# mattiaskvist/yolo-v1

Measured on AMD Instinct MI355X. Metric: images/sec at 448x448, forward (YOLOv1Backbone + FC head), higher is better.
Workload: dtype bf16; 1 GPU; BASELINE.json configs[1]: batch=64/GPU 448x448 forward-only, YOLOv1Backbone + FC head, 1xMI355X per rank; global_batch=64, per_gpu_batch=64, weights=random init (torch default, seed 0), parallelism=single

## Files before the change

include/yolo_hip.h:

```cpp
#ifndef YOLO_HIP_H
#define YOLO_HIP_H

#include <stddef.h>
#include <stdint.h>

#ifdef __cplusplus
extern "C" {
#endif

#define YOLO_HIP_ABI_VERSION 2

#define YOLO_E_ARG (-1)
#define YOLO_E_UNSUPPORTED (-2)

typedef void *yolo_stream_t;

int yolo_hip_abi_version(void);
const char *yolo_hip_last_error(void);
int yolo_debug_stamps(void *buf, int k_iter);
int yolo_stream_create(int low, yolo_stream_t *out);


int yolo_decode(const float *pred, int N, int S, int B, int C, double conf_thr,
                double *rec, int32_t *counts, yolo_stream_t stream);
// ... 91 lines not shown
int yolo_maxpool2_bwd_codes(const yolo_pool_desc *d, const void *ypool_bf16, const void *codes_u16, const void *dpool_bf16,
                            float slope, void *dz_bf16, yolo_stream_t stream);


int yolo_nchw_f32_to_nhwc_bf16(const float *x, int N, int C, int H, int W, void *y, int Cpad,
                               int halo_lo, int halo_hi, yolo_stream_t stream);
int yolo_nhwc_bf16_to_nchw_f32(const void *x, int N, int C, int H, int W, int halo, float *y, yolo_stream_t stream);
int yolo_nhwc_bf16_to_nchw_bf16(const void *x, int N, int C, int H, int W, int halo, void *y, yolo_stream_t stream);

int yolo_pack_conv_weight(const float *w_oihw, int Cout, int Cin, int KH, int KW, int Cinp, int KWp,
                          void *w_fwd_bf16, void *w_dgrad_bf16, yolo_stream_t stream);
int yolo_pack_fc_weight(const float *w, int O, int C, int HW, void *w_fwd_bf16, void *w_t_bf16, yolo_stream_t stream);
int yolo_pack_fc_weight_blocked(const float *w, int O, long K, void *w_panels_bf16, yolo_stream_t stream);
int yolo_pack_fc_weight_blocked_hwc(const float *w, int O, int C, int HW, void *w_panels_bf16, yolo_stream_t stream);
int yolo_unpack_conv_wgrad(const float *dw_packed, int Cout, int Cin, int KH, int KW, int Cinp, int KWp,
                           float *dw_oihw, int accumulate, yolo_stream_t stream);
int yolo_conv_stem7_fwd(const void *x_nhwc4_bf16, const void *w_packed_bf16, const float *bias, int N, int Ho, int Wo,
                        long x_img_stride, int x_row_stride, float slope, int pool2, void *out_bf16,
                        long out_img_stride, int out_row_stride, int out_off, void *out_full_bf16,
                        long full_img_stride, int full_row_stride, int full_off, yolo_stream_t stream);
int yolo_conv_stem7_fwd_f32(const float *x_nchw_f32, const void *w_packed_bf16, const float *bias, int N, int H, int W, float slope,
                            int pool2, void *out_bf16, long out_img_stride, int out_row_stride, int out_off, void *out_full_bf16,
                            long full_img_stride, int full_row_stride, int full_off, yolo_stream_t stream);
int yolo_wgrad_stem7(const void *x_nhwc4_bf16, const void *dy_bf16, int N, int Ho, int Wo, long x_img_stride,
                     int x_row_stride, long dy_img_stride, int dy_row_stride, int dy_off, float *dw_oihw,
                     float *db, float *scratch, long scratch_elems, yolo_stream_t stream);
int yolo_wgrad_stem7_pooled(const void *x_nhwc4_bf16, const void *y_full_bf16, int N, int Ho, int Wo, long x_img_stride,
                            int x_row_stride, long y_img_stride, int y_row_stride, int y_off, const void *dpool_bf16,
                            long dp_img_stride, int dp_row_stride, int dp_off, float slope, float *dw_oihw, float *db,
                            float *scratch, long scratch_elems, yolo_stream_t stream);
int yolo_wgrad_stem7_codes(const void *x_nhwc4_bf16, const void *y_pooled_bf16, const void *codes_u16, int N, int Ho, int Wo,
                           long x_img_stride, int x_row_stride, const void *dpool_bf16, long dp_img_stride, int dp_row_stride,
                           int dp_off, float slope, float *dw_oihw, float *db, float *scratch, long scratch_elems,
                           yolo_stream_t stream);
#define YOLO_PACK_MAX 32
typedef struct yolo_conv_pack_item {
    const float *w;
    void *w_fwd_bf16;
    void *w_dgrad_bf16;
    int Cout, Cin, KH, KW;
} yolo_conv_pack_item;
typedef struct yolo_conv_unpack_item {
    const float *dw_packed;
    float *dw_oihw;
    int Cout, Cin, KH, KW;
} yolo_conv_unpack_item;
// ... 122 lines not shown
```

yolo-v1_amd/csrc/stem.hip:

```cpp
#include <algorithm>

#include "common.h"

namespace yolo {

typedef __attribute__((ext_vector_type(8))) __bf16 sbf16x8;
typedef __attribute__((ext_vector_type(4))) float sf32x4;

#define STEM_GLDS16(gptr, lptr) \
    __builtin_amdgcn_global_load_lds((const __attribute__((address_space(1))) void *)(gptr), (__attribute__((address_space(3))) void *)(lptr), 16, 0, 0)

constexpr int SF_TH = 8, SF_TW = 16;
constexpr int SF_PW = 40, SF_PH = 21;
constexpr int SF_X_BYTES = 7 * 1024;
constexpr int SF_OP = 64 + 8;
constexpr int SF_OUT_BYTES = SF_TH * SF_TW * SF_OP * 2;

struct StemFwdParams {
    const bf16_t *x;
    const bf16_t *w;
    const float *bias;
    bf16_t *out;
    int tiles_x, tiles_y, ntiles;
    long x_img_stride, out_img_stride;
    int x_row_stride, out_row_stride, out_off;
    int pool;
    float slope;
    bf16_t *full;
    unsigned short *codes;
    long full_img_stride;
    int full_row_stride, full_off;
    const float *x32;
    int H, W;
};

template <bool F32IN>
__global__ void __launch_bounds__(256, 2) stem_fwd_kernel(const StemFwdParams p)
{
    __shared__ __attribute__((aligned(16))) char patchA[SF_X_BYTES];
    __shared__ __attribute__((aligned(16))) char patchB[SF_X_BYTES];
    __shared__ __attribute__((aligned(16))) bf16_t otileA[SF_TH * SF_TW * SF_OP];
    __shared__ __attribute__((aligned(16))) bf16_t otileB[SF_TH * SF_TW * SF_OP];
    const int tid = threadIdx.x, lane = tid & 63;
    const int wave = __builtin_amdgcn_readfirstlane(tid >> 6);
    const int n16 = lane & 15, kb = lane >> 4;

    sbf16x8 afrag[4][7];
#pragma unroll
    for (int mb = 0; mb < 4; ++mb)
#pragma unroll
        for (int ky = 0; ky < 7; ++ky)
            afrag[mb][ky] = *reinterpret_cast<const sbf16x8 *>(p.w + ((mb * 16 + n16) * 7 + ky) * 32 + kb * 8);
    float bias_r[4][4];
#pragma unroll
    for (int mb = 0; mb < 4; ++mb)
#pragma unroll
        for (int r = 0; r < 4; ++r) bias_r[mb][r] = p.bias[mb * 16 + 4 * kb + r];

    int x_off[2];
#pragma unroll
    for (int i = 0; i < 2; ++i) {
        int slot = (i * 4 + wave) * 64 + lane;
        if (slot >= SF_PH * (SF_PW / 2)) slot = SF_PH * (SF_PW / 2) - 1;
        x_off[i] = (slot / (SF_PW / 2)) * p.x_row_stride + (slot % (SF_PW / 2)) * 8;
    }
    auto stage = [&](char *sb, int tile) {
        const int tx = tile % p.tiles_x, r = tile / p.tiles_x;
        const int ty = r % p.tiles_y, n = r / p.tiles_y;
        const bf16_t *xb = p.x + (long)n * p.x_img_stride + (long)(ty * SF_TH * 2) * p.x_row_stride + tx * SF_TW * 2 * 4;
        STEM_GLDS16(xb + x_off[0], sb + wave * 1024);
        if (wave < 3) STEM_GLDS16(xb + x_off[1], sb + (4 + wave) * 1024);
    };

    constexpr int F32_ITEMS = SF_PH * 3 * 11, F32_PER_THREAD = (F32_ITEMS + 255) / 256;
    float4 xr[F32_PER_THREAD];
    if constexpr (F32IN) {
        for (int i = tid; i < SF_X_BYTES / 16; i += 256) {
            *reinterpret_cast<uint4 *>(patchA + i * 16) = uint4{0u, 0u, 0u, 0u};
            *reinterpret_cast<uint4 *>(patchB + i * 16) = uint4{0u, 0u, 0u, 0u};
        }
        __syncthreads();
    }
    auto f32_load = [&](int tile) {
        const int tx = tile % p.tiles_x, r = tile / p.tiles_x;
        const int ty = r % p.tiles_y, n = r / p.tiles_y;
        const float *xb = p.x32 + (long)n * 3 * p.H * p.W;
#pragma unroll
        for (int j = 0; j < F32_PER_THREAD; ++j) {
            const int item = j * 256 + tid;
            const int q = item % 11, rc = item / 11, c = rc % 3, pr = rc / 3;
            const int y = ty * SF_TH * 2 - 3 + pr, x = tx * SF_TW * 2 - 4 + 4 * q;
            const bool in = item < F32_ITEMS && y >= 0 && y < p.H && x >= 0 && x < p.W;
            xr[j] = in ? *reinterpret_cast<const float4 *>(xb + ((long)c * p.H + y) * p.W + x) : float4{0.0f, 0.0f, 0.0f, 0.0f};
        }
    };
    auto f32_store = [&](char *sb) {
#pragma unroll
        for (int j = 0; j < F32_PER_THREAD; ++j) {
            const int item = j * 256 + tid;
            if (item >= F32_ITEMS) continue;
            const int q = item % 11, rc = item / 11, c = rc % 3, pr = rc / 3;
            const float v[4] = {xr[j].x, xr[j].y, xr[j].z, xr[j].w};
#pragma unroll
            for (int e = 0; e < 4; ++e) {
                const int ppx = 4 * q - 1 + e;
                if (ppx >= 0 && ppx < SF_PW) *reinterpret_cast<bf16_t *>(sb + (pr * SF_PW + ppx) * 8 + c * 2) = f32_to_bf16(v[e]);
            }
        }
    };

    const int b_base = ((4 * wave) * SF_PW + 2 * n16 + 2 * kb) * 8;

    auto mfma_phase = [&](const char *sb, bf16_t *otile) {
        sf32x4 acc[4][2];
#pragma unroll
        for (int mb = 0; mb < 4; ++mb)
#pragma unroll
            for (int rr = 0; rr < 2; ++rr) acc[mb][rr] = sf32x4{0.0f, 0.0f, 0.0f, 0.0f};
#pragma unroll
        for (int ky = 0; ky < 7; ++ky) {
            sbf16x8 bfr[2];
#pragma unroll
            for (int rr = 0; rr < 2; ++rr) bfr[rr] = *reinterpret_cast<const sbf16x8 *>(sb + b_base + ((2 * rr + ky) * SF_PW) * 8);
#pragma unroll
            for (int mb = 0; mb < 4; ++mb)
#pragma unroll
                for (int rr = 0; rr < 2; ++rr) acc[mb][rr] = __builtin_amdgcn_mfma_f32_16x16x32_bf16(afrag[mb][ky], bfr[rr], acc[mb][rr], 0, 0, 0);
        }
#pragma unroll
        for (int rr = 0; rr < 2; ++rr) {
            const int px = (2 * wave + rr) * SF_TW + n16;
#pragma unroll
            for (int mb = 0; mb < 4; ++mb) {
                float v[4];
#pragma unroll
                for (int r = 0; r < 4; ++r) {
                    v[r] = acc[mb][rr][r] + bias_r[mb][r];
                    v[r] = v[r] > 0.0f ? v[r] : v[r] * p.slope;
                }
                uint2 o;
                o.x = (unsigned)f32_to_bf16(v[0]) | ((unsigned)f32_to_bf16(v[1]) << 16);
                o.y = (unsigned)f32_to_bf16(v[2]) | ((unsigned)f32_to_bf16(v[3]) << 16);
                *reinterpret_cast<uint2 *>(otile + px * SF_OP + mb * 16 + 4 * kb) = o;
            }
        }
    };
    auto store_phase = [&](const bf16_t *otile, int tile) {
        const int tx = tile % p.tiles_x, r0 = tile / p.tiles_x;
        const int ty = r0 % p.tiles_y, n = r0 / p.tiles_y;
        bf16_t *ob = p.out + (long)n * p.out_img_stride + p.out_off;
        if (p.pool) {
            const int c8 = tid & 7, q = tid >> 3, qy = q >> 3, qx = q & 7;
            const bf16_t *s0 = otile + ((2 * qy) * SF_TW + 2 * qx) * SF_OP + c8 * 8;
            const uint4 a = *reinterpret_cast<const uint4 *>(s0), b = *reinterpret_cast<const uint4 *>(s0 + SF_OP);
            const uint4 c = *reinterpret_cast<const uint4 *>(s0 + SF_TW * SF_OP), d = *reinterpret_cast<const uint4 *>(s0 + SF_TW * SF_OP + SF_OP);
            const unsigned va[4] = {a.x, a.y, a.z, a.w}, vb[4] = {b.x, b.y, b.z, b.w}, vc[4] = {c.x, c.y, c.z, c.w}, vd[4] = {d.x, d.y, d.z, d.w};
            unsigned o[4];
#pragma unroll
            for (int k = 0; k < 4; ++k) {
                const float lo = fmaxf(fmaxf(__uint_as_float(va[k] << 16), __uint_as_float(vb[k] << 16)), fmaxf(__uint_as_float(vc[k] << 16), __uint_as_float(vd[k] << 16)));
                const float hi = fmaxf(fmaxf(__uint_as_float(va[k] & 0xffff0000u), __uint_as_float(vb[k] & 0xffff0000u)),
                                       fmaxf(__uint_as_float(vc[k] & 0xffff0000u), __uint_as_float(vd[k] & 0xffff0000u)));
                o[k] = (__float_as_uint(lo) >> 16) | (__float_as_uint(hi) & 0xffff0000u);
            }
            const long pa = (long)(ty * (SF_TH / 2) + qy) * p.out_row_stride + (tx * (SF_TW / 2) + qx) * 64 + c8 * 8;
            *reinterpret_cast<uint4 *>(ob + pa) = uint4{o[0], o[1], o[2], o[3]};
            if (p.codes) {
                unsigned code = 0;
#pragma unroll
                for (int k = 0; k < 4; ++k) {
#pragma unroll
                    for (int hf = 0; hf < 2; ++hf) {
                        const float w0 = hf ? __uint_as_float(va[k] & 0xffff0000u) : __uint_as_float(va[k] << 16);
                        const float w1 = hf ? __uint_as_float(vb[k] & 0xffff0000u) : __uint_as_float(vb[k] << 16);
                        const float w2 = hf ? __uint_as_float(vc[k] & 0xffff0000u) : __uint_as_float(vc[k] << 16);
                        const float w3 = hf ? __uint_as_float(vd[k] & 0xffff0000u) : __uint_as_float(vd[k] << 16);
                        unsigned am = 0;
                        float m = w0;
                        if (w1 > m) { m = w1; am = 1; }
                        if (w2 > m) { m = w2; am = 2; }
                        if (w3 > m) { m = w3; am = 3; }
                        code |= am << (2 * (2 * k + hf));
                    }
                }
                p.codes[((long)n * p.out_img_stride + p.out_off + pa) >> 3] = (unsigned short)code;
            }
            if (p.full) {
                bf16_t *fb = p.full + (long)n * p.full_img_stride + p.full_off;
#pragma unroll
                for (int pass = 0; pass < 4; ++pass) {
                    const int idx = pass * 256 + tid, cc = idx & 7, px = idx >> 3;
                    const uint4 v = *reinterpret_cast<const uint4 *>(otile + px * SF_OP + cc * 8);
                    *reinterpret_cast<uint4 *>(fb + (long)(ty * SF_TH + (px >> 4)) * p.full_row_stride + (tx * SF_TW + (px & 15)) * 64 + cc * 8) = v;
                }
            }
        } else {
#pragma unroll
            for (int pass = 0; pass < 4; ++pass) {
                const int idx = pass * 256 + tid, c8 = idx & 7, px = idx >> 3;
                const int py = px >> 4, pxx = px & 15;
                const uint4 v = *reinterpret_cast<const uint4 *>(otile + px * SF_OP + c8 * 8);
                *reinterpret_cast<uint4 *>(ob + (long)(ty * SF_TH + py) * p.out_row_stride + (tx * SF_TW + pxx) * 64 + c8 * 8) = v;
            }
        }
    };

    const int G = gridDim.x;
    int tile = blockIdx.x, prev = -1;
    if (tile < p.ntiles) {
        if constexpr (F32IN) {
            f32_load(tile);
            f32_store(patchA);
        } else {
            stage(patchA, tile);
        }
    }
    while (tile < p.ntiles) {
        asm volatile("s_waitcnt vmcnt(0) lgkmcnt(0)" ::: "memory");
        __builtin_amdgcn_s_barrier();
        asm volatile("" ::: "memory");
        if (tile + G < p.ntiles) {
            if constexpr (F32IN) f32_load(tile + G);
            else stage(patchB, tile + G);
        }
        if (prev >= 0) store_phase(otileB, prev);
        mfma_phase(patchA, otileA);
        if constexpr (F32IN) {
            if (tile + G < p.ntiles) f32_store(patchB);
// ... 10 lines not shown
        asm volatile("s_waitcnt vmcnt(0) lgkmcnt(0)" ::: "memory");
        __builtin_amdgcn_s_barrier();
        asm volatile("" ::: "memory");
        if (tile + G < p.ntiles) {
            if constexpr (F32IN) f32_load(tile + G);
            else stage(patchA, tile + G);
        }
        store_phase(otileA, prev);
        mfma_phase(patchB, otileB);
        if constexpr (F32IN) {
            if (tile + G < p.ntiles) f32_store(patchA);
        }
        prev = tile;
        tile += G;
        if (tile >= p.ntiles) {
            asm volatile("s_waitcnt lgkmcnt(0)" ::: "memory");
            __builtin_amdgcn_s_barrier();
            asm volatile("" ::: "memory");
            store_phase(otileB, prev);
        }
    }
}

}

using namespace yolo;

YOLO_API int yolo_conv_stem7_fwd(const void *x_nhwc4, const void *w_packed, const float *bias, int N, int Ho, int Wo, long x_img_stride, int x_row_stride,
                                 float slope, int pool2, void *out, long out_img_stride, int out_row_stride, int out_off, void *out_full, long full_img_stride,
                                 int full_row_stride, int full_off, yolo_stream_t stream)
{
    if (pool2 == 3 && !out_full) return fail(YOLO_E_ARG, "yolo_conv_stem7_fwd: pool2 = 3 writes the arg-max codes through out_full");
    if (out_full && pool2 != 3 && (!pool2 || (full_row_stride & 7) || (full_img_stride & 7) || (full_off & 7) || ((uintptr_t)out_full & 15)))
        return fail(YOLO_E_ARG, "yolo_conv_stem7_fwd: out_full needs pool2 = 1 and strides in multiples of 8 elements");
    if (!x_nhwc4 || !w_packed || !bias || !out || N <= 0 || Ho <= 0 || Wo <= 0) return fail(YOLO_E_ARG, "yolo_conv_stem7_fwd: bad argument");
    if ((Ho % SF_TH) || (Wo % SF_TW)) return fail(YOLO_E_UNSUPPORTED, "yolo_conv_stem7_fwd: output %dx%d is not a multiple of %dx%d (use yolo_igemm)", Ho, Wo, SF_TH, SF_TW);
    if ((x_row_stride & 7) || (x_img_stride & 7) || (out_row_stride & 7) || (out_img_stride & 7) || (out_off & 7) || ((uintptr_t)x_nhwc4 & 15) || ((uintptr_t)out & 15) ||
        ((uintptr_t)w_packed & 15))
        return fail(YOLO_E_UNSUPPORTED, "yolo_conv_stem7_fwd: strides must be multiples of 8 elements and pointers 16-B aligned");
    StemFwdParams p{};
    p.x = (const bf16_t *)x_nhwc4; p.w = (const bf16_t *)w_packed; p.bias = bias; p.out = (bf16_t *)out;
    p.tiles_x = Wo / SF_TW; p.tiles_y = Ho / SF_TH;
    const long nt = (long)N * p.tiles_x * p.tiles_y;
    if (nt > 0x7fffffffL) return fail(YOLO_E_UNSUPPORTED, "yolo_conv_stem7_fwd: too many tiles");
    p.ntiles = (int)nt;
    p.x_img_stride = x_img_stride; p.out_img_stride = out_img_stride;
    p.x_row_stride = x_row_stride; p.out_row_stride = out_row_stride; p.out_off = out_off;
    p.pool = pool2 ? 1 : 0;
    p.slope = slope;
    if (pool2 == 3) {
        p.codes = (unsigned short *)out_full;
    } else {
        p.full = (bf16_t *)out_full; p.full_img_stride = full_img_stride; p.full_row_stride = full_row_stride; p.full_off = full_off;
    }
    const long G = std::min<long>(nt, 1024);
    hipLaunchKernelGGL(stem_fwd_kernel<false>, dim3((unsigned)G), dim3(256), 0, STRM(stream), p);
    return check_launch("yolo_conv_stem7_fwd");
}

YOLO_API int yolo_conv_stem7_fwd_f32(const float *x_nchw, const void *w_packed, const float *bias, int N, int H, int W, float slope, int pool2, void *out,
                                     long out_img_stride, int out_row_stride, int out_off, void *out_full, long full_img_stride, int full_row_stride, int full_off,
                                     yolo_stream_t stream)
{
    const int Ho = H / 2, Wo = W / 2;
    if (!x_nchw || !w_packed || !bias || !out || N <= 0 || H <= 0 || W <= 0 || (H & 1) || (W & 1)) return fail(YOLO_E_ARG, "yolo_conv_stem7_fwd_f32: bad argument");
    if (pool2 == 3 && !out_full) return fail(YOLO_E_ARG, "yolo_conv_stem7_fwd_f32: pool2 = 3 writes the arg-max codes through out_full");
    if (out_full && pool2 != 3 && (!pool2 || (full_row_stride & 7) || (full_img_stride & 7) || (full_off & 7) || ((uintptr_t)out_full & 15)))
        return fail(YOLO_E_ARG, "yolo_conv_stem7_fwd_f32: out_full needs pool2 = 1 and strides in multiples of 8 elements");
    if ((Ho % SF_TH) || (Wo % SF_TW)) return fail(YOLO_E_UNSUPPORTED, "yolo_conv_stem7_fwd_f32: output %dx%d is not a multiple of %dx%d", Ho, Wo, SF_TH, SF_TW);
    if ((uintptr_t)x_nchw & 15) return fail(YOLO_E_UNSUPPORTED, "yolo_conv_stem7_fwd_f32: the input must be 16-B aligned (rows are read as float4)");
    if ((out_row_stride & 7) || (out_img_stride & 7) || (out_off & 7) || ((uintptr_t)out & 15) || ((uintptr_t)w_packed & 15))
        return fail(YOLO_E_UNSUPPORTED, "yolo_conv_stem7_fwd_f32: strides must be multiples of 8 elements and pointers 16-B aligned");
    StemFwdParams p{};
    p.x32 = x_nchw; p.H = H; p.W = W;
    p.w = (const bf16_t *)w_packed; p.bias = bias; p.out = (bf16_t *)out;
    p.tiles_x = Wo / SF_TW; p.tiles_y = Ho / SF_TH;
    const long nt = (long)N * p.tiles_x * p.tiles_y;
    if (nt > 0x7fffffffL) return fail(YOLO_E_UNSUPPORTED, "yolo_conv_stem7_fwd_f32: too many tiles");
    p.ntiles = (int)nt;
    p.out_img_stride = out_img_stride; p.out_row_stride = out_row_stride; p.out_off = out_off;
    p.pool = pool2 ? 1 : 0;
    p.slope = slope;
    if (pool2 == 3) {
        p.codes = (unsigned short *)out_full;
    } else {
        p.full = (bf16_t *)out_full; p.full_img_stride = full_img_stride; p.full_row_stride = full_row_stride; p.full_off = full_off;
    }
    const long G = std::min<long>(nt, 1024);
    hipLaunchKernelGGL(stem_fwd_kernel<true>, dim3((unsigned)G), dim3(256), 0, STRM(stream), p);
    return check_launch("yolo_conv_stem7_fwd_f32");
}
```

yolo-v1_amd/yolo/_hip.py:

```python

from __future__ import annotations

import ctypes
import os

import torch

_HERE = os.path.dirname(os.path.abspath(__file__))
LIB_PATH = os.environ.get("YOLO_HIP_LIB") or os.path.join(_HERE, "libyolo_hip.so")
_LIB = None

ABI_VERSION = 2
BN_ACC_REPLICAS = 16
c_int, c_long, c_float, c_double, c_void_p = ctypes.c_int, ctypes.c_long, ctypes.c_float, ctypes.c_double, ctypes.c_void_p


class IgemmDesc(ctypes.Structure):

    _fields_ = [
        ("N", ctypes.c_int32), ("Ho", ctypes.c_int32), ("Wo", ctypes.c_int32),
        ("in_img_stride", ctypes.c_int64),
        ("in_row_stride", ctypes.c_int32), ("in_px_stride", ctypes.c_int32), ("in_off", ctypes.c_int32),
        ("stride", ctypes.c_int32), ("KH", ctypes.c_int32), ("KW", ctypes.c_int32),
        ("tap_len", ctypes.c_int32), ("Cout", ctypes.c_int32),
# ... 79 lines not shown
    "yolo_hip_abi_version": [],
    "yolo_debug_stamps": [c_void_p, c_int],
    "yolo_stream_create": [c_int, ctypes.POINTER(c_void_p)],
    "yolo_decode": [c_void_p, c_int, c_int, c_int, c_int, c_double, c_void_p, c_void_p, c_void_p],
    "yolo_decode_gt": [c_void_p, c_int, c_int, c_int, c_int, c_void_p, c_void_p, c_void_p],
    "yolo_nms": [c_void_p, c_void_p, c_int, c_int, c_double, c_int, c_void_p, c_void_p, c_void_p],
    "yolo_batchnorm_train_fwd": [c_void_p, c_int, c_int, c_int, c_int, c_int, c_void_p, c_void_p, c_double, c_double, c_void_p, c_void_p, c_void_p, c_int,
                                 c_int, c_void_p, c_void_p, c_void_p, c_int, c_void_p, c_int, c_void_p],
    "yolo_batchnorm_bwd": [c_void_p, c_int, c_void_p, c_int, c_void_p, c_int, c_int, c_int, c_int, c_int, c_void_p, c_void_p, c_void_p, ctypes.c_long, ctypes.c_long,
                           ctypes.c_long, ctypes.c_long, c_int, c_int, c_void_p, c_void_p, c_void_p, c_void_p, c_void_p],
    "yolo_map_match": [c_void_p, c_void_p, c_void_p, c_int, c_int, c_void_p, c_void_p, c_int, ctypes.POINTER(c_double), c_int, c_double, c_double, c_double,
                       c_void_p, c_void_p, c_void_p],
    "yolo_pairwise_iou": [c_void_p, c_int, c_void_p, c_int, c_int, c_void_p, c_void_p],
    "yolo_loss_fwd_bwd": [c_void_p, c_void_p, c_int, c_int, c_int, c_int, c_float, c_float, c_void_p, c_void_p, c_void_p, c_void_p],
    "yolo_loss_iou": [c_void_p, c_void_p, c_long, c_void_p, c_void_p],
    "yolo_igemm": [ctypes.POINTER(IgemmDesc), c_void_p, c_void_p, c_void_p, c_void_p, c_void_p, c_void_p],
    "yolo_igemm_finish": [ctypes.POINTER(IgemmDesc), c_void_p, c_void_p, c_void_p, c_void_p, c_void_p],
    "yolo_wgrad": [ctypes.POINTER(WgradDesc), c_void_p, c_void_p, c_void_p, c_void_p, c_void_p],
    "yolo_wgrad_slab_floats": [ctypes.POINTER(WgradDesc), ctypes.POINTER(ctypes.c_long)],
    "yolo_conv_stem7_fwd": [c_void_p, c_void_p, c_void_p, c_int, c_int, c_int, c_long, c_int, c_float, c_int, c_void_p, c_long, c_int, c_int, c_void_p, c_long,
                            c_int, c_int, c_void_p],
    "yolo_conv_stem7_fwd_f32": [c_void_p, c_void_p, c_void_p, c_int, c_int, c_int, c_float, c_int, c_void_p, c_long, c_int, c_int, c_void_p, c_long, c_int, c_int,
                                c_void_p],
    "yolo_wgrad_stem7": [c_void_p, c_void_p, c_int, c_int, c_int, c_long, c_int, c_long, c_int, c_int, c_void_p, c_void_p, c_void_p, c_long, c_void_p],
    "yolo_wgrad_stem7_pooled": [c_void_p, c_void_p, c_int, c_int, c_int, c_long, c_int, c_long, c_int, c_int, c_void_p, c_long, c_int, c_int, c_float, c_void_p,
                                c_void_p, c_void_p, c_long, c_void_p],
    "yolo_wgrad_stem7_codes": [c_void_p, c_void_p, c_void_p, c_int, c_int, c_int, c_long, c_int, c_void_p, c_long, c_int, c_int, c_float, c_void_p, c_void_p, c_void_p,
                               c_long, c_void_p],
    "yolo_maxpool3s2_fwd": [ctypes.POINTER(PoolDesc), c_void_p, c_void_p, c_void_p],
    "yolo_maxpool3s2_bwd": [ctypes.POINTER(PoolDesc), c_void_p, c_void_p, c_void_p, c_int, c_void_p],
    "yolo_maxpool2_fwd": [ctypes.POINTER(PoolDesc), c_void_p, c_void_p, c_void_p],
    "yolo_maxpool2_bwd_lrelu": [ctypes.POINTER(PoolDesc), c_void_p, c_void_p, c_float, c_void_p, c_void_p],
    "yolo_maxpool2_bwd_codes": [ctypes.POINTER(PoolDesc), c_void_p, c_void_p, c_void_p, c_float, c_void_p, c_void_p],
    "yolo_nchw_f32_to_nhwc_bf16": [c_void_p, c_int, c_int, c_int, c_int, c_void_p, c_int, c_int, c_int, c_void_p],
    "yolo_nhwc_bf16_to_nchw_f32": [c_void_p, c_int, c_int, c_int, c_int, c_int, c_void_p, c_void_p],
    "yolo_nhwc_bf16_to_nchw_bf16": [c_void_p, c_int, c_int, c_int, c_int, c_int, c_void_p, c_void_p],
    "yolo_scale_rows_to_bf16": [c_void_p, c_void_p, c_float, c_void_p, c_float, c_int, c_int, c_int, c_void_p, c_void_p],
    "yolo_dropout_bf16": [c_void_p, c_void_p, c_float, c_long, c_void_p, c_void_p],
    "yolo_pack_conv_weight": [c_void_p, c_int, c_int, c_int, c_int, c_int, c_int, c_void_p, c_void_p, c_void_p],
    "yolo_pack_fc_weight": [c_void_p, c_int, c_int, c_int, c_void_p, c_void_p, c_void_p],
    "yolo_pack_fc_weight_blocked": [c_void_p, c_int, c_long, c_void_p, c_void_p],
    "yolo_pack_fc_weight_blocked_hwc": [c_void_p, c_int, c_int, c_int, c_void_p, c_void_p],
    "yolo_unpack_conv_wgrad": [c_void_p, c_int, c_int, c_int, c_int, c_int, c_int, c_void_p, c_int, c_void_p],
    "yolo_im2col_rows": [c_void_p, c_long, c_int, c_int, c_int, c_int, c_int, c_int, c_int, c_int, c_int, c_void_p, c_void_p],
    "yolo_transpose_f32_to_bf16": [c_void_p, c_int, c_int, c_void_p, c_int, c_void_p],
    "yolo_transpose_bf16": [c_void_p, c_int, c_int, c_int, c_void_p, c_int, c_void_p],
# ... 115 lines not shown
```

yolo-v1_amd/yolo/config.py:

```python

from __future__ import annotations

from dataclasses import dataclass, fields


@dataclass
class EngineConfig:
    TIMERS: list | None = None
    IGEMM_LAUNCHES: int = 0
    TUNE_LOG: list | None = None
    AUTOTUNE: bool = False
    TILE_HINT: int = 0
    TILE_PX: int = 0
    PLAN_TABLE: bool = True
    BORROW_PLANS: bool = True
    SMALL_SPLIT: bool = True
    PERSIST: bool = True
    BN_STATS_IN_CONV: bool = True
    STEM_KERNEL: bool = True
    STEM_POOL_BWD_FUSED: bool = True
    STRIDE2_CLASSES: bool = True
    STEM_F32_INPUT: bool = True
    FLATTEN_FREE: bool = True
    POOL_CODES: bool = True
    FUSE_POOL: bool = True
    FC_NORM_IN_WGRAD: int = 1 << 26
    WGRAD_STREAM: bool = True
    SIDE_LOW: bool = True
    WGRAD_SLABS: bool = False
    WGRAD_PIPE: bool = True
    WGRAD_CHOICE: object = None
    PLAN_TIMES: object = None
    TUNE_REPS: int = 1
    FC_WGRAD_SIDE: bool = True
    DETERMINISTIC: bool = False
    WGRAD_WIDE: bool = True


def _from_env(cfg: EngineConfig) -> EngineConfig:
    import os
    for f in fields(EngineConfig):
        v = os.environ.get("YOLO_AMD_" + f.name)
        if v is None:
            continue
        if f.type not in ("bool", "int"):
            raise ValueError(f"YOLO_AMD_{f.name}: only the bool / int switches can be set from the environment")
        setattr(cfg, f.name, bool(int(v)) if f.type == "bool" else int(v))
    return cfg


CONFIG = _from_env(EngineConfig())
SWITCHES = frozenset(f.name for f in fields(EngineConfig))
```

Measured before the change: 24370 images/s.

## Add 16-row stem conv tile kernel with in-register 2x2 pooling path

Adds a new stem 7x7 conv forward kernel that processes 16 output rows per tile instead of 8. This amortizes halo loads across more rows and reduces the tile count, and it launches with a smaller grid. When pooling is requested without codes or full output and the slope is non-negative, a variant does the 2x2 maxpool in registers using DPP lane swaps, which skips the LDS output tile round-trip. A host-side rule selects the new kernel based on tile count, with an override knob. The trade-offs are more LDS per block, higher register pressure and less parallelism for small batches.

```diff
diff --git a/include/yolo_hip.h b/include/yolo_hip.h
--- a/include/yolo_hip.h
+++ b/include/yolo_hip.h
@@ -137,6 +137,7 @@
 int yolo_conv_stem7_fwd_f32(const float *x_nchw_f32, const void *w_packed_bf16, const float *bias, int N, int H, int W, float slope,
                             int pool2, void *out_bf16, long out_img_stride, int out_row_stride, int out_off, void *out_full_bf16,
                             long full_img_stride, int full_row_stride, int full_off, yolo_stream_t stream);
+int yolo_conv_stem7_set_tile(int tile_rows);
 int yolo_wgrad_stem7(const void *x_nhwc4_bf16, const void *dy_bf16, int N, int Ho, int Wo, long x_img_stride,
                      int x_row_stride, long dy_img_stride, int dy_row_stride, int dy_off, float *dw_oihw,
                      float *db, float *scratch, long scratch_elems, yolo_stream_t stream);
diff --git a/yolo-v1_amd/csrc/stem.hip b/yolo-v1_amd/csrc/stem.hip
--- a/yolo-v1_amd/csrc/stem.hip
+++ b/yolo-v1_amd/csrc/stem.hip
@@ -1,4 +1,5 @@
 #include <algorithm>
+#include <atomic>
 
 #include "common.h"
 
@@ -34,123 +35,16 @@
     int H, W;
 };
 
-template <bool F32IN>
-__global__ void __launch_bounds__(256, 2) stem_fwd_kernel(const StemFwdParams p)
-{
-    __shared__ __attribute__((aligned(16))) char patchA[SF_X_BYTES];
-    __shared__ __attribute__((aligned(16))) char patchB[SF_X_BYTES];
-    __shared__ __attribute__((aligned(16))) bf16_t otileA[SF_TH * SF_TW * SF_OP];
-    __shared__ __attribute__((aligned(16))) bf16_t otileB[SF_TH * SF_TW * SF_OP];
-    const int tid = threadIdx.x, lane = tid & 63;
-    const int wave = __builtin_amdgcn_readfirstlane(tid >> 6);
-    const int n16 = lane & 15, kb = lane >> 4;
-
-    sbf16x8 afrag[4][7];
-#pragma unroll
-    for (int mb = 0; mb < 4; ++mb)
-#pragma unroll
-        for (int ky = 0; ky < 7; ++ky)
-            afrag[mb][ky] = *reinterpret_cast<const sbf16x8 *>(p.w + ((mb * 16 + n16) * 7 + ky) * 32 + kb * 8);
-    float bias_r[4][4];
-#pragma unroll
-    for (int mb = 0; mb < 4; ++mb)
-#pragma unroll
-        for (int r = 0; r < 4; ++r) bias_r[mb][r] = p.bias[mb * 16 + 4 * kb + r];
-
-    int x_off[2];
-#pragma unroll
-    for (int i = 0; i < 2; ++i) {
-        int slot = (i * 4 + wave) * 64 + lane;
-        if (slot >= SF_PH * (SF_PW / 2)) slot = SF_PH * (SF_PW / 2) - 1;
-        x_off[i] = (slot / (SF_PW / 2)) * p.x_row_stride + (slot % (SF_PW / 2)) * 8;
-    }
-    auto stage = [&](char *sb, int tile) {
-        const int tx = tile % p.tiles_x, r = tile / p.tiles_x;
-        const int ty = r % p.tiles_y, n = r / p.tiles_y;
-        const bf16_t *xb = p.x + (long)n * p.x_img_stride + (long)(ty * SF_TH * 2) * p.x_row_stride + tx * SF_TW * 2 * 4;
-        STEM_GLDS16(xb + x_off[0], sb + wave * 1024);
-        if (wave < 3) STEM_GLDS16(xb + x_off[1], sb + (4 + wave) * 1024);
-    };
-
-    constexpr int F32_ITEMS = SF_PH * 3 * 11, F32_PER_THREAD = (F32_ITEMS + 255) / 256;
-    float4 xr[F32_PER_THREAD];
-    if constexpr (F32IN) {
-        for (int i = tid; i < SF_X_BYTES / 16; i += 256) {
-            *reinterpret_cast<uint4 *>(patchA + i * 16) = uint4{0u, 0u, 0u, 0u};
-            *reinterpret_cast<uint4 *>(patchB + i * 16) = uint4{0u, 0u, 0u, 0u};
-        }
-        __syncthreads();
-    }
-    auto f32_load = [&](int tile) {
-        const int tx = tile % p.tiles_x, r = tile / p.tiles_x;
-        const int ty = r % p.tiles_y, n = r / p.tiles_y;
-        const float *xb = p.x32 + (long)n * 3 * p.H * p.W;
-#pragma unroll
-        for (int j = 0; j < F32_PER_THREAD; ++j) {
-            const int item = j * 256 + tid;
-            const int q = item % 11, rc = item / 11, c = rc % 3, pr = rc / 3;
-            const int y = ty * SF_TH * 2 - 3 + pr, x = tx * SF_TW * 2 - 4 + 4 * q;
-            const bool in = item < F32_ITEMS && y >= 0 && y < p.H && x >= 0 && x < p.W;
-            xr[j] = in ? *reinterpret_cast<const float4 *>(xb + ((long)c * p.H + y) * p.W + x) : float4{0.0f, 0.0f, 0.0f, 0.0f};
-        }
-    };
-    auto f32_store = [&](char *sb) {
-#pragma unroll
-        for (int j = 0; j < F32_PER_THREAD; ++j) {
-            const int item = j * 256 + tid;
-            if (item >= F32_ITEMS) continue;
-            const int q = item % 11, rc = item / 11, c = rc % 3, pr = rc / 3;
-            const float v[4] = {xr[j].x, xr[j].y, xr[j].z, xr[j].w};
-#pragma unroll
-            for (int e = 0; e < 4; ++e) {
-                const int ppx = 4 * q - 1 + e;
-                if (ppx >= 0 && ppx < SF_PW) *reinterpret_cast<bf16_t *>(sb + (pr * SF_PW + ppx) * 8 + c * 2) = f32_to_bf16(v[e]);
-            }
-        }
-    };
-
-    const int b_base = ((4 * wave) * SF_PW + 2 * n16 + 2 * kb) * 8;
-
-    auto mfma_phase = [&](const char *sb, bf16_t *otile) {
-        sf32x4 acc[4][2];
-#pragma unroll
-        for (int mb = 0; mb < 4; ++mb)
-#pragma unroll
-            for (int rr = 0; rr < 2; ++rr) acc[mb][rr] = sf32x4{0.0f, 0.0f, 0.0f, 0.0f};
-#pragma unroll
-        for (int ky = 0; ky < 7; ++ky) {
-            sbf16x8 bfr[2];
-#pragma unroll
-            for (int rr = 0; rr < 2; ++rr) bfr[rr] = *reinterpret_cast<const sbf16x8 *>(sb + b_base + ((2 * rr + ky) * SF_PW) * 8);
-#pragma unroll
-            for (int mb = 0; mb < 4; ++mb)
-#pragma unroll
-                for (int rr = 0; rr < 2; ++rr) acc[mb][rr] = __builtin_amdgcn_mfma_f32_16x16x32_bf16(afrag[mb][ky], bfr[rr], acc[mb][rr], 0, 0, 0);
-        }
-#pragma unroll
-        for (int rr = 0; rr < 2; ++rr) {
-            const int px = (2 * wave + rr) * SF_TW + n16;
-#pragma unroll
-            for (int mb = 0; mb < 4; ++mb) {
-                float v[4];
-#pragma unroll
-                for (int r = 0; r < 4; ++r) {
-                    v[r] = acc[mb][rr][r] + bias_r[mb][r];
-                    v[r] = v[r] > 0.0f ? v[r] : v[r] * p.slope;
-                }
-                uint2 o;
-                o.x = (unsigned)f32_to_bf16(v[0]) | ((unsigned)f32_to_bf16(v[1]) << 16);
-                o.y = (unsigned)f32_to_bf16(v[2]) | ((unsigned)f32_to_bf16(v[3]) << 16);
-                *reinterpret_cast<uint2 *>(otile + px * SF_OP + mb * 16 + 4 * kb) = o;
-            }
-        }
-    };
-    auto store_phase = [&](const bf16_t *otile, int tile) {
-        const int tx = tile % p.tiles_x, r0 = tile / p.tiles_x;
-        const int ty = r0 % p.tiles_y, n = r0 / p.tiles_y;
-        bf16_t *ob = p.out + (long)n * p.out_img_stride + p.out_off;
-        if (p.pool) {
-            const int c8 = tid & 7, q = tid >> 3, qy = q >> 3, qx = q & 7;
+template <int TH>
+__device__ __forceinline__ void stem_store_tile(const StemFwdParams &p, const bf16_t *otile, int tile, int tid)
+{
+    const int tx = tile % p.tiles_x, r0 = tile / p.tiles_x;
+    const int ty = r0 % p.tiles_y, n = r0 / p.tiles_y;
+    bf16_t *ob = p.out + (long)n * p.out_img_stride + p.out_off;
+    if (p.pool) {
+#pragma unroll
+        for (int pass = 0; pass < TH / 8; ++pass) {
+            const int idx = pass * 256 + tid, c8 = idx & 7, q = idx >> 3, qy = q >> 3, qx = q & 7;
             const bf16_t *s0 = otile + ((2 * qy) * SF_TW + 2 * qx) * SF_OP + c8 * 8;
             const uint4 a = *reinterpret_cast<const uint4 *>(s0), b = *reinterpret_cast<const uint4 *>(s0 + SF_OP);
             const uint4 c = *reinterpret_cast<const uint4 *>(s0 + SF_TW * SF_OP), d = *reinterpret_cast<const uint4 *>(s0 + SF_TW * SF_OP + SF_OP);
@@ -163,7 +57,7 @@
                                        fmaxf(__uint_as_float(vc[k] & 0xffff0000u), __uint_as_float(vd[k] & 0xffff0000u)));
                 o[k] = (__float_as_uint(lo) >> 16) | (__float_as_uint(hi) & 0xffff0000u);
             }
-            const long pa = (long)(ty * (SF_TH / 2) + qy) * p.out_row_stride + (tx * (SF_TW / 2) + qx) * 64 + c8 * 8;
+            const long pa = (long)(ty * (TH / 2) + qy) * p.out_row_stride + (tx * (SF_TW / 2) + qx) * 64 + c8 * 8;
             *reinterpret_cast<uint4 *>(ob + pa) = uint4{o[0], o[1], o[2], o[3]};
             if (p.codes) {
                 unsigned code = 0;
@@ -185,25 +79,139 @@
                 }
                 p.codes[((long)n * p.out_img_stride + p.out_off + pa) >> 3] = (unsigned short)code;
             }
-            if (p.full) {
-                bf16_t *fb = p.full + (long)n * p.full_img_stride + p.full_off;
-#pragma unroll
-                for (int pass = 0; pass < 4; ++pass) {
-                    const int idx = pass * 256 + tid, cc = idx & 7, px = idx >> 3;
-                    const uint4 v = *reinterpret_cast<const uint4 *>(otile + px * SF_OP + cc * 8);
-                    *reinterpret_cast<uint4 *>(fb + (long)(ty * SF_TH + (px >> 4)) * p.full_row_stride + (tx * SF_TW + (px & 15)) * 64 + cc * 8) = v;
+        }
+        if (p.full) {
+            bf16_t *fb = p.full + (long)n * p.full_img_stride + p.full_off;
+#pragma unroll
+            for (int pass = 0; pass < TH / 2; ++pass) {
+                const int idx = pass * 256 + tid, cc = idx & 7, px = idx >> 3;
+                const uint4 v = *reinterpret_cast<const uint4 *>(otile + px * SF_OP + cc * 8);
+                *reinterpret_cast<uint4 *>(fb + (long)(ty * TH + (px >> 4)) * p.full_row_stride + (tx * SF_TW + (px & 15)) * 64 + cc * 8) = v;
+            }
+        }
+    } else {
+#pragma unroll
+        for (int pass = 0; pass < TH / 2; ++pass) {
+            const int idx = pass * 256 + tid, c8 = idx & 7, px = idx >> 3;
+            const int py = px >> 4, pxx = px & 15;
+            const uint4 v = *reinterpret_cast<const uint4 *>(otile + px * SF_OP + c8 * 8);
+            *reinterpret_cast<uint4 *>(ob + (long)(ty * TH + py) * p.out_row_stride + (tx * SF_TW + pxx) * 64 + c8 * 8) = v;
+        }
+    }
+}
+
+template <bool F32IN>
+__global__ void __launch_bounds__(256, 2) stem_fwd_kernel(const StemFwdParams p)
+{
+    __shared__ __attribute__((aligned(16))) char patchA[SF_X_BYTES];
+    __shared__ __attribute__((aligned(16))) char patchB[SF_X_BYTES];
+    __shared__ __attribute__((aligned(16))) bf16_t otileA[SF_TH * SF_TW * SF_OP];
+    __shared__ __attribute__((aligned(16))) bf16_t otileB[SF_TH * SF_TW * SF_OP];
+    const int tid = threadIdx.x, lane = tid & 63;
+    const int wave = __builtin_amdgcn_readfirstlane(tid >> 6);
+    const int n16 = lane & 15, kb = lane >> 4;
+
+    sbf16x8 afrag[4][7];
+#pragma unroll
+    for (int mb = 0; mb < 4; ++mb)
+#pragma unroll
+        for (int ky = 0; ky < 7; ++ky)
+            afrag[mb][ky] = *reinterpret_cast<const sbf16x8 *>(p.w + ((mb * 16 + n16) * 7 + ky) * 32 + kb * 8);
+    float bias_r[4][4];
+#pragma unroll
+    for (int mb = 0; mb < 4; ++mb)
+#pragma unroll
+        for (int r = 0; r < 4; ++r) bias_r[mb][r] = p.bias[mb * 16 + 4 * kb + r];
+
+    int x_off[2];
+#pragma unroll
+    for (int i = 0; i < 2; ++i) {
+        int slot = (i * 4 + wave) * 64 + lane;
+        if (slot >= SF_PH * (SF_PW / 2)) slot = SF_PH * (SF_PW / 2) - 1;
+        x_off[i] = (slot / (SF_PW / 2)) * p.x_row_stride + (slot % (SF_PW / 2)) * 8;
+    }
+    auto stage = [&](char *sb, int tile) {
+        const int tx = tile % p.tiles_x, r = tile / p.tiles_x;
+        const int ty = r % p.tiles_y, n = r / p.tiles_y;
+        const bf16_t *xb = p.x + (long)n * p.x_img_stride + (long)(ty * SF_TH * 2) * p.x_row_stride + tx * SF_TW * 2 * 4;
+        STEM_GLDS16(xb + x_off[0], sb + wave * 1024);
+        if (wave < 3) STEM_GLDS16(xb + x_off[1], sb + (4 + wave) * 1024);
+    };
+
+    constexpr int F32_ITEMS = SF_PH * 3 * 11, F32_PER_THREAD = (F32_ITEMS + 255) / 256;
+    float4 xr[F32_PER_THREAD];
+    if constexpr (F32IN) {
+        for (int i = tid; i < SF_X_BYTES / 16; i += 256) {
+            *reinterpret_cast<uint4 *>(patchA + i * 16) = uint4{0u, 0u, 0u, 0u};
+            *reinterpret_cast<uint4 *>(patchB + i * 16) = uint4{0u, 0u, 0u, 0u};
+        }
+        __syncthreads();
+    }
+    auto f32_load = [&](int tile) {
+        const int tx = tile % p.tiles_x, r = tile / p.tiles_x;
+        const int ty = r % p.tiles_y, n = r / p.tiles_y;
+        const float *xb = p.x32 + (long)n * 3 * p.H * p.W;
+#pragma unroll
+        for (int j = 0; j < F32_PER_THREAD; ++j) {
+            const int item = j * 256 + tid;
+            const int q = item % 11, rc = item / 11, c = rc % 3, pr = rc / 3;
+            const int y = ty * SF_TH * 2 - 3 + pr, x = tx * SF_TW * 2 - 4 + 4 * q;
+            const bool in = item < F32_ITEMS && y >= 0 && y < p.H && x >= 0 && x < p.W;
+            xr[j] = in ? *reinterpret_cast<const float4 *>(xb + ((long)c * p.H + y) * p.W + x) : float4{0.0f, 0.0f, 0.0f, 0.0f};
+        }
+    };
+    auto f32_store = [&](char *sb) {
+#pragma unroll
+        for (int j = 0; j < F32_PER_THREAD; ++j) {
+            const int item = j * 256 + tid;
+            if (item >= F32_ITEMS) continue;
+            const int q = item % 11, rc = item / 11, c = rc % 3, pr = rc / 3;
+            const float v[4] = {xr[j].x, xr[j].y, xr[j].z, xr[j].w};
+#pragma unroll
+            for (int e = 0; e < 4; ++e) {
+                const int ppx = 4 * q - 1 + e;
+                if (ppx >= 0 && ppx < SF_PW) *reinterpret_cast<bf16_t *>(sb + (pr * SF_PW + ppx) * 8 + c * 2) = f32_to_bf16(v[e]);
+            }
+        }
+    };
+
+    const int b_base = ((4 * wave) * SF_PW + 2 * n16 + 2 * kb) * 8;
+
+    auto mfma_phase = [&](const char *sb, bf16_t *otile) {
+        sf32x4 acc[4][2];
+#pragma unroll
+        for (int mb = 0; mb < 4; ++mb)
+#pragma unroll
+            for (int rr = 0; rr < 2; ++rr) acc[mb][rr] = sf32x4{0.0f, 0.0f, 0.0f, 0.0f};
+#pragma unroll
+        for (int ky = 0; ky < 7; ++ky) {
+            sbf16x8 bfr[2];
+#pragma unroll
+            for (int rr = 0; rr < 2; ++rr) bfr[rr] = *reinterpret_cast<const sbf16x8 *>(sb + b_base + ((2 * rr + ky) * SF_PW) * 8);
+#pragma unroll
+            for (int mb = 0; mb < 4; ++mb)
+#pragma unroll
+                for (int rr = 0; rr < 2; ++rr) acc[mb][rr] = __builtin_amdgcn_mfma_f32_16x16x32_bf16(afrag[mb][ky], bfr[rr], acc[mb][rr], 0, 0, 0);
+        }
+#pragma unroll
+        for (int rr = 0; rr < 2; ++rr) {
+            const int px = (2 * wave + rr) * SF_TW + n16;
+#pragma unroll
+            for (int mb = 0; mb < 4; ++mb) {
+                float v[4];
+#pragma unroll
+                for (int r = 0; r < 4; ++r) {
+                    v[r] = acc[mb][rr][r] + bias_r[mb][r];
+                    v[r] = v[r] > 0.0f ? v[r] : v[r] * p.slope;
                 }
-            }
-        } else {
-#pragma unroll
-            for (int pass = 0; pass < 4; ++pass) {
-                const int idx = pass * 256 + tid, c8 = idx & 7, px = idx >> 3;
-                const int py = px >> 4, pxx = px & 15;
-                const uint4 v = *reinterpret_cast<const uint4 *>(otile + px * SF_OP + c8 * 8);
-                *reinterpret_cast<uint4 *>(ob + (long)(ty * SF_TH + py) * p.out_row_stride + (tx * SF_TW + pxx) * 64 + c8 * 8) = v;
-            }
-        }
-    };
+                uint2 o;
+                o.x = (unsigned)f32_to_bf16(v[0]) | ((unsigned)f32_to_bf16(v[1]) << 16);
+                o.y = (unsigned)f32_to_bf16(v[2]) | ((unsigned)f32_to_bf16(v[3]) << 16);
+                *reinterpret_cast<uint2 *>(otile + px * SF_OP + mb * 16 + 4 * kb) = o;
+            }
+        }
+    };
+    auto store_phase = [&](const bf16_t *otile, int tile) { stem_store_tile<SF_TH>(p, otile, tile, tid); };
 
     const int G = gridDim.x;
     int tile = blockIdx.x, prev = -1;
@@ -260,9 +268,239 @@
     }
 }
 
+constexpr int S16_TH = 16;
+constexpr int S16_PH = 2 * S16_TH + 5;
+constexpr int S16_X_BYTES = 12 * 1024;
+constexpr int S16_QUADS = 10;
+
+template <bool F32IN, bool REGPOOL>
+__global__ void __launch_bounds__(256, 2) stem_fwd16_kernel(const StemFwdParams p)
+{
+    __shared__ __attribute__((aligned(16))) char patch[2 * S16_X_BYTES];
+    __shared__ __attribute__((aligned(16))) bf16_t otile[REGPOOL ? 8 : S16_TH * SF_TW * SF_OP];
+    __shared__ __attribute__((aligned(16))) float bias_s[64];
+    const int tid = threadIdx.x, lane = tid & 63;
+    const int wave = __builtin_amdgcn_readfirstlane(tid >> 6);
+    const int n16 = lane & 15, kb = lane >> 4;
+
+    sbf16x8 afrag[4][7];
+#pragma unroll
+    for (int mb = 0; mb < 4; ++mb)
+#pragma unroll
+        for (int ky = 0; ky < 7; ++ky)
+            afrag[mb][ky] = *reinterpret_cast<const sbf16x8 *>(p.w + ((mb * 16 + n16) * 7 + ky) * 32 + kb * 8);
+    if (tid < 64) bias_s[tid] = p.bias[tid];
+
+    int x_off[3];
+#pragma unroll
+    for (int i = 0; i < 3; ++i) {
+        int slot = (i * 4 + wave) * 64 + lane;
+        if (slot >= S16_PH * (SF_PW / 2)) slot = S16_PH * (SF_PW / 2) - 1;
+        x_off[i] = (slot / (SF_PW / 2)) * p.x_row_stride + (slot % (SF_PW / 2)) * 8;
+    }
+    auto stage = [&](char *sb, int tile) {
+        const int tx = tile % p.tiles_x, r = tile / p.tiles_x;
+        const int ty = r % p.tiles_y, n = r / p.tiles_y;
+        const bf16_t *xb = p.x + (long)n * p.x_img_stride + (long)(ty * S16_TH * 2) * p.x_row_stride + tx * SF_TW * 2 * 4;
+#pragma unroll
+        for (int i = 0; i < 3; ++i) STEM_GLDS16(xb + x_off[i], sb + (i * 4 + wave) * 1024);
+    };
+
+    constexpr int F32_ITEMS = S16_PH * S16_QUADS, F32_PER_THREAD = (F32_ITEMS + 255) / 256;
+    float4 xr[F32_PER_THREAD][3];
+    auto f32_load = [&](int tile) {
+        const int tx = tile % p.tiles_x, r = tile / p.tiles_x;
+        const int ty = r % p.tiles_y, n = r / p.tiles_y;
+        const float *xb = p.x32 + (long)n * 3 * p.H * p.W;
+#pragma unroll
+        for (int j = 0; j < F32_PER_THREAD; ++j) {
+            const int item = j * 256 + tid;
+            const int q = item % S16_QUADS, pr = item / S16_QUADS;
+            const int y = ty * S16_TH * 2 - 3 + pr, x = tx * SF_TW * 2 - 4 + 4 * q;
+            const bool in = item < F32_ITEMS && y >= 0 && y < p.H && x >= 0 && x < p.W;
+#pragma unroll
+            for (int c = 0; c < 3; ++c)
+                xr[j][c] = in ? *reinterpret_cast<const float4 *>(xb + ((long)c * p.H + y) * p.W + x) : float4{0.0f, 0.0f, 0.0f, 0.0f};
+        }
+    };
+    auto f32_store = [&](char *sb) {
+#pragma unroll
+        for (int j = 0; j < F32_PER_THREAD; ++j) {
+            const int item = j * 256 + tid;
+            if (item >= F32_ITEMS) continue;
+            const int q = item % S16_QUADS, pr = item / S16_QUADS;
+            const float v[3][4] = {{xr[j][0].x, xr[j][0].y, xr[j][0].z, xr[j][0].w}, {xr[j][1].x, xr[j][1].y, xr[j][1].z, xr[j][1].w},
+                                   {xr[j][2].x, xr[j][2].y, xr[j][2].z, xr[j][2].w}};
+#pragma unroll
+            for (int e = 0; e < 4; ++e) {
+                const int ppx = 4 * q - 1 + e;
+                if (ppx < 0) continue;
+                uint2 o;
+                o.x = (unsigned)f32_to_bf16(v[0][e]) | ((unsigned)f32_to_bf16(v[1][e]) << 16);
+                o.y = (unsigned)f32_to_bf16(v[2][e]);
+                *reinterpret_cast<uint2 *>(sb + (pr * SF_PW + ppx) * 8) = o;
+            }
+        }
+    };
+
+    const int b_base = ((8 * wave) * SF_PW + 2 * n16 + 2 * kb) * 8;
+
+    const int G = gridDim.x;
+    int tile = blockIdx.x, prev = -1, buf = 0;
+    if (tile < p.ntiles) {
+        if constexpr (F32IN) {
+            f32_load(tile);
+            f32_store(patch);
+        } else {
+            stage(patch, tile);
+        }
+    }
+    while (tile < p.ntiles) {
+        if constexpr (F32IN) asm volatile("s_waitcnt lgkmcnt(0)" ::: "memory");
+        else asm volatile("s_waitcnt vmcnt(0) lgkmcnt(0)" ::: "memory");
+        __builtin_amdgcn_s_barrier();
+        asm volatile("" ::: "memory");
+        const char *sb = patch + buf * S16_X_BYTES;
+        char *sn = patch + (buf ^ 1) * S16_X_BYTES;
+        const bool more = tile + G < p.ntiles;
+        if constexpr (!REGPOOL) {
+            if (prev >= 0) stem_store_tile<S16_TH>(p, otile, prev, tid);
+        }
+        if (more) {
+            if constexpr (F32IN) f32_load(tile + G);
+            else stage(sn, tile + G);
+        }
+
+        sf32x4 acc[4][4];
+#pragma unroll
+        for (int mb = 0; mb < 4; ++mb)
+#pragma unroll
+            for (int rr = 0; rr < 4; ++rr) acc[mb][rr] = sf32x4{0.0f, 0.0f, 0.0f, 0.0f};
+#pragma unroll
+        for (int j = 0; j < 13; ++j) {
+            const sbf16x8 bfr = *reinterpret_cast<const sbf16x8 *>(sb + b_base + (j * SF_PW) * 8);
+#pragma unroll
+            for (int rr = 0; rr < 4; ++rr) {
+                const int ky = j - 2 * rr;
+                if (ky < 0 || ky >= 7) continue;
+#pragma unroll
+                for (int mb = 0; mb < 4; ++mb) acc[mb][rr] = __builtin_amdgcn_mfma_f32_16x16x32_bf16(afrag[mb][ky], bfr, acc[mb][rr], 0, 0, 0);
+            }
+        }
+
+        __builtin_amdgcn_sched_barrier(0);
+        if constexpr (REGPOOL) {
+            const int tx = tile % p.tiles_x, r0 = tile / p.tiles_x;
+            const int ty = r0 % p.tiles_y, n = r0 / p.tiles_y;
+            const int h = lane & 1;
+            bf16_t *ob = p.out + (long)n * p.out_img_stride + p.out_off + (tx * (SF_TW / 2) + (n16 >> 1)) * 64 + 4 * kb;
+#pragma unroll
+            for (int pr = 0; pr < 2; ++pr) {
+                bf16_t *orow = ob + (long)(ty * (S16_TH / 2) + 2 * wave + pr) * p.out_row_stride;
+#pragma unroll
+                for (int i = 0; i < 2; ++i) {
+                    const int mbh = 2 * i + h;
+                    const float4 bs = *reinterpret_cast<const float4 *>(bias_s + mbh * 16 + 4 * kb);
+                    const float bv[4] = {bs.x, bs.y, bs.z, bs.w};
+                    float v[4];
+#pragma unroll
+                    for (int r = 0; r < 4; ++r) {
+                        float m0 = fmaxf(acc[2 * i][2 * pr][r], acc[2 * i][2 * pr + 1][r]);
+                        float m1 = fmaxf(acc[2 * i + 1][2 * pr][r], acc[2 * i + 1][2 * pr + 1][r]);
+                        m0 = fmaxf(m0, __int_as_float(__builtin_amdgcn_update_dpp(0, __float_as_int(m0), 0xB1, 0xF, 0xF, true)));
+                        m1 = fmaxf(m1, __int_as_float(__builtin_amdgcn_update_dpp(0, __float_as_int(m1), 0xB1, 0xF, 0xF, true)));
+                        v[r] = (h ? m1 : m0) + bv[r];
+                        v[r] = v[r] > 0.0f ? v[r] : v[r] * p.slope;
+                    }
+                    uint2 o;
+                    o.x = (unsigned)f32_to_bf16(v[0]) | ((unsigned)f32_to_bf16(v[1]) << 16);
+                    o.y = (unsigned)f32_to_bf16(v[2]) | ((unsigned)f32_to_bf16(v[3]) << 16);
+                    *reinterpret_cast<uint2 *>(orow + mbh * 16) = o;
+                }
+            }
+        } else {
+            asm volatile("s_waitcnt lgkmcnt(0)" ::: "memory");
+            __builtin_amdgcn_s_barrier();
+            asm volatile("" ::: "memory");
+#pragma unroll
+            for (int rr = 0; rr < 4; ++rr) {
+                const int px = (4 * wave + rr) * SF_TW + n16;
+#pragma unroll
+                for (int mb = 0; mb < 4; ++mb) {
+                    const float4 bs = *reinterpret_cast<const float4 *>(bias_s + mb * 16 + 4 * kb);
+                    const float bv[4] = {bs.x, bs.y, bs.z, bs.w};
+                    float v[4];
+#pragma unroll
+                    for (int r = 0; r < 4; ++r) {
+                        v[r] = acc[mb][rr][r] + bv[r];
+                        v[r] = v[r] > 0.0f ? v[r] : v[r] * p.slope;
+                    }
+                    uint2 o;
+                    o.x = (unsigned)f32_to_bf16(v[0]) | ((unsigned)f32_to_bf16(v[1]) << 16);
+                    o.y = (unsigned)f32_to_bf16(v[2]) | ((unsigned)f32_to_bf16(v[3]) << 16);
+                    *reinterpret_cast<uint2 *>(otile + px * SF_OP + mb * 16 + 4 * kb) = o;
+                }
+            }
+        }
+        if constexpr (F32IN) {
+            if (more) f32_store(sn);
+        }
+        prev = tile;
+        tile += G;
+        buf ^= 1;
+    }
+    if constexpr (!REGPOOL) {
+        if (prev >= 0) {
+            asm volatile("s_waitcnt lgkmcnt(0)" ::: "memory");
+            __builtin_amdgcn_s_barrier();
+            asm volatile("" ::: "memory");
+            stem_store_tile<S16_TH>(p, otile, prev, tid);
+        }
+    }
+}
+
+static std::atomic<int> g_stem_tile{0};
+constexpr long S16_MIN_TILES = 196;
+constexpr long S16_GRID = 512;
+
+static bool stem_use_tile16(int N, int Ho, int Wo)
+{
+    if ((Ho % S16_TH) || (Wo % SF_TW)) return false;
+    const int forced = g_stem_tile.load(std::memory_order_relaxed);
+    if (forced) return forced == S16_TH;
+    return (long)N * (Ho / S16_TH) * (Wo / SF_TW) >= S16_MIN_TILES;
+}
+
+template <bool F32IN>
+static int stem_launch(StemFwdParams &p, int N, int Ho, int Wo, hipStream_t stream, const char *what)
+{
+    const bool t16 = stem_use_tile16(N, Ho, Wo);
+    const int th = t16 ? S16_TH : SF_TH;
+    p.tiles_x = Wo / SF_TW; p.tiles_y = Ho / th;
+    const long nt = (long)N * p.tiles_x * p.tiles_y;
+    if (nt > 0x7fffffffL) return fail(YOLO_E_UNSUPPORTED, "%s: too many tiles", what);
+    p.ntiles = (int)nt;
+    if (t16) {
+        const long G = std::min<long>(nt, S16_GRID);
+        if (p.pool && !p.full && !p.codes && p.slope >= 0.0f) hipLaunchKernelGGL((stem_fwd16_kernel<F32IN, true>), dim3((unsigned)G), dim3(256), 0, stream, p);
+        else hipLaunchKernelGGL((stem_fwd16_kernel<F32IN, false>), dim3((unsigned)G), dim3(256), 0, stream, p);
+    } else {
+        const long G = std::min<long>(nt, 1024);
+        hipLaunchKernelGGL(stem_fwd_kernel<F32IN>, dim3((unsigned)G), dim3(256), 0, stream, p);
+    }
+    return check_launch(what);
+}
+
 }
 
 using namespace yolo;
+
+YOLO_API int yolo_conv_stem7_set_tile(int tile_rows)
+{
+    if (tile_rows != 0 && tile_rows != SF_TH && tile_rows != S16_TH) return fail(YOLO_E_ARG, "yolo_conv_stem7_set_tile: 0 (the rule), 8 or 16, not %d", tile_rows);
+    g_stem_tile.store(tile_rows, std::memory_order_relaxed);
+    return 0;
+}
 
 YOLO_API int yolo_conv_stem7_fwd(const void *x_nhwc4, const void *w_packed, const float *bias, int N, int Ho, int Wo, long x_img_stride, int x_row_stride,
                                  float slope, int pool2, void *out, long out_img_stride, int out_row_stride, int out_off, void *out_full, long full_img_stride,
@@ -278,10 +516,6 @@
         return fail(YOLO_E_UNSUPPORTED, "yolo_conv_stem7_fwd: strides must be multiples of 8 elements and pointers 16-B aligned");
     StemFwdParams p{};
     p.x = (const bf16_t *)x_nhwc4; p.w = (const bf16_t *)w_packed; p.bias = bias; p.out = (bf16_t *)out;
-    p.tiles_x = Wo / SF_TW; p.tiles_y = Ho / SF_TH;
-    const long nt = (long)N * p.tiles_x * p.tiles_y;
-    if (nt > 0x7fffffffL) return fail(YOLO_E_UNSUPPORTED, "yolo_conv_stem7_fwd: too many tiles");
-    p.ntiles = (int)nt;
     p.x_img_stride = x_img_stride; p.out_img_stride = out_img_stride;
     p.x_row_stride = x_row_stride; p.out_row_stride = out_row_stride; p.out_off = out_off;
     p.pool = pool2 ? 1 : 0;
@@ -291,9 +525,7 @@
     } else {
         p.full = (bf16_t *)out_full; p.full_img_stride = full_img_stride; p.full_row_stride = full_row_stride; p.full_off = full_off;
     }
-    const long G = std::min<long>(nt, 1024);
-    hipLaunchKernelGGL(stem_fwd_kernel<false>, dim3((unsigned)G), dim3(256), 0, STRM(stream), p);
-    return check_launch("yolo_conv_stem7_fwd");
+    return stem_launch<false>(p, N, Ho, Wo, STRM(stream), "yolo_conv_stem7_fwd");
 }
 
 YOLO_API int yolo_conv_stem7_fwd_f32(const float *x_nchw, const void *w_packed, const float *bias, int N, int H, int W, float slope, int pool2, void *out,
@@ -312,10 +544,6 @@
     StemFwdParams p{};
     p.x32 = x_nchw; p.H = H; p.W = W;
     p.w = (const bf16_t *)w_packed; p.bias = bias; p.out = (bf16_t *)out;
-    p.tiles_x = Wo / SF_TW; p.tiles_y = Ho / SF_TH;
-    const long nt = (long)N * p.tiles_x * p.tiles_y;
-    if (nt > 0x7fffffffL) return fail(YOLO_E_UNSUPPORTED, "yolo_conv_stem7_fwd_f32: too many tiles");
-    p.ntiles = (int)nt;
     p.out_img_stride = out_img_stride; p.out_row_stride = out_row_stride; p.out_off = out_off;
     p.pool = pool2 ? 1 : 0;
     p.slope = slope;
@@ -324,7 +552,5 @@
     } else {
         p.full = (bf16_t *)out_full; p.full_img_stride = full_img_stride; p.full_row_stride = full_row_stride; p.full_off = full_off;
     }
-    const long G = std::min<long>(nt, 1024);
-    hipLaunchKernelGGL(stem_fwd_kernel<true>, dim3((unsigned)G), dim3(256), 0, STRM(stream), p);
-    return check_launch("yolo_conv_stem7_fwd_f32");
-}
+    return stem_launch<true>(p, N, Ho, Wo, STRM(stream), "yolo_conv_stem7_fwd_f32");
+}
diff --git a/yolo-v1_amd/yolo/_hip.py b/yolo-v1_amd/yolo/_hip.py
--- a/yolo-v1_amd/yolo/_hip.py
+++ b/yolo-v1_amd/yolo/_hip.py
@@ -125,6 +125,7 @@
                             c_int, c_int, c_void_p],
     "yolo_conv_stem7_fwd_f32": [c_void_p, c_void_p, c_void_p, c_int, c_int, c_int, c_float, c_int, c_void_p, c_long, c_int, c_int, c_void_p, c_long, c_int, c_int,
                                 c_void_p],
+    "yolo_conv_stem7_set_tile": [c_int],
     "yolo_wgrad_stem7": [c_void_p, c_void_p, c_int, c_int, c_int, c_long, c_int, c_long, c_int, c_int, c_void_p, c_void_p, c_void_p, c_long, c_void_p],
     "yolo_wgrad_stem7_pooled": [c_void_p, c_void_p, c_int, c_int, c_int, c_long, c_int, c_long, c_int, c_int, c_void_p, c_long, c_int, c_int, c_float, c_void_p,
                                 c_void_p, c_void_p, c_long, c_void_p],
diff --git a/yolo-v1_amd/yolo/config.py b/yolo-v1_amd/yolo/config.py
--- a/yolo-v1_amd/yolo/config.py
+++ b/yolo-v1_amd/yolo/config.py
@@ -18,6 +18,7 @@
     PERSIST: bool = True
     BN_STATS_IN_CONV: bool = True
     STEM_KERNEL: bool = True
+    STEM_TILE: int = 0
     STEM_POOL_BWD_FUSED: bool = True
     STRIDE2_CLASSES: bool = True
     STEM_F32_INPUT: bool = True
@@ -37,6 +38,13 @@
     WGRAD_WIDE: bool = True
 
 
+    def __setattr__(self, name, value):
+        if name == "STEM_TILE" and int(value) != getattr(self, "STEM_TILE", 0):
+            from . import _hip
+            _hip.check(_hip.lib().yolo_conv_stem7_set_tile(int(value)), "conv_stem7_set_tile")
+        object.__setattr__(self, name, value)
+
+
 def _from_env(cfg: EngineConfig) -> EngineConfig:
     import os
     for f in fields(EngineConfig):
```

Result: no change. 24600 images/s, median of 6 (+1.0%).
